# aynik/carta1

Measured on AMD Instinct MI355X. Metric: atrac1_stereo_frames_per_s_encode, higher is better.
Workload: dtype f32+f64

## Files before the change

### carta1_amd/csrc/c1_k_allocate.hip

```cpp
#include "c1_device.h"

namespace {

constexpr int kHeapSlotsPerLane = 52 + 1;
constexpr uint32_t kLow = 0x1FFFFFu;
constexpr uint32_t kSentinel = 52u;
constexpr int kCandBytes = kCandidateBytes;
constexpr double kAlive = -1.0;

__device__ __forceinline__ uint32_t heap_entry(uint32_t rank, int size, int s, int wl, int b) {
  return (rank << 21) | ((uint32_t)size << 16) | ((uint32_t)s << 10) | ((uint32_t)wl << 6) | (uint32_t)b;
}

__device__ __forceinline__ void heap_sift_down(uint32_t *hp, int sentinel, int i, uint32_t v, uint32_t el,
                                               uint32_t er, bool active) {
  const uint32_t vmax = v | kLow;
  for (;;) {
    const uint32_t m = max(el | kLow, vmax);
    const bool take_r = er > m;
    const bool take_l = !take_r && el > vmax;
    const bool moved = active && (take_r || take_l);
    if (active) hp[i * 64] = moved ? (take_r ? er : el) : v;
    active = moved;
    if (__builtin_amdgcn_ballot_w64(active) == 0) break;
    i = moved ? 2 * i + 1 + (take_r ? 1 : 0) : i;
    const int l = 2 * i + 1;
    const uint32_t *src = hp + min(l, sentinel - 1) * 64;
    el = l < sentinel ? src[0] : 0u;
    er = src[64];
  }
}

constexpr int kSpecsHost[52] = {8, 8, 8, 8, 4, 4, 4, 4, 8, 8, 8, 8, 6, 6, 6, 6, 6, 6, 6, 6, 6, 6, 6, 6, 7, 7, 7, 7, 9, 9, 9, 9, 10, 10, 10, 10,
                                12, 12, 12, 12, 12, 12, 12, 12, 20, 20, 20, 20, 20, 20, 20, 20};
constexpr int dist_class(int size) {
  for (int c = 0; c < 8; c++) if (kDistSizes[c] == size) return c;
  return -1;
}
constexpr bool sizes_come_in_fours() {
  for (int b = 0; b < 52; b++) if (kSpecsHost[b] != kSpecsHost[b & ~3]) return false;
  return true;
}
static_assert(sizes_come_in_fours(), "the four BFUs whose indices share a dword share a size");
static_assert(dist_class(4) == 0 && dist_class(20) == 7 && dist_class(kSpecsHost[24]) == 2, "every BFU size has its row of the distortion tables");

__device__ __forceinline__ void reopen(uint32_t (&sf)[13]) {
#pragma unroll
  for (int i = 0; i < 13; i++) asm volatile("" : "+v"(sf[i]));
}

template <bool AFFINE>
__device__ __forceinline__ void heap_phase(uint32_t *hp, int n, const uint32_t (&sf)[13], const C1DevEncOpts *O, bool live) {
  const __attribute__((address_space(4))) uint16_t *rank_t = (const __attribute__((address_space(4))) uint16_t *)O->rank;
  const uint32_t mul0 = ((uint32_t)O->rank_a << 11) | 1u, add0 = (uint32_t)(O->rank_c + O->rank_off) << 11;
  const uint32_t step0 = O->rank_step0, step = O->rank_step;
  int remaining = 212 * 8 - 40 - 10 * n;
  int hs = 0;
#pragma unroll
  for (int b0 = 0; b0 < 52; b0 += 13) if (own_block()) {
#pragma unroll
  for (int b = b0; b < b0 + 13; b++) {
    if (b < n) {
      const int s = (sf[b >> 2] >> ((b & 3) * 8)) & 63;
      const uint32_t fixed = ((uint32_t)kSpecsHost[b] << 16) | (uint32_t)b;
      if constexpr (AFFINE) hp[hs * 64] = ((__umul24(mul0, (uint32_t)s) + add0) << 10) | fixed;
      else hp[hs * 64] = ((uint32_t)rank_t[s * 16] << 21) | ((uint32_t)s << 10) | fixed;
      hs += (s != 0 && live) ? 1 : 0;
    }
  }
  }
  for (int k = hs; k < kHeapSlotsPerLane; k++) hp[k * 64] = kSentinel;
  for (int i = (hs >> 1) - 1; i >= 0; i--) {
    const int l = 2 * i + 1;
    heap_sift_down(hp, 52, i, hp[i * 64], hp[l * 64], hp[(l + 1) * 64], true);
  }
  uint32_t r0 = hp[0], r1 = hp[64], r2 = hp[128];
  bool run = remaining >= 4 && hs > 0;
  while (__builtin_amdgcn_ballot_w64(run) != 0) {
    const uint32_t top = r0;
    const bool wl0 = (top & (15u << 6)) == 0;
    const int size = (top >> 16) & 31;
    const int cost = size << (wl0 ? 1 : 0);
    const bool fits = cost <= remaining;
    uint32_t v, upd;
    bool last_wl;
    if constexpr (AFFINE) {
      v = top + (wl0 ? step0 : step);
      upd = (fits ? v : top) & kLow;
      last_wl = (v & (15u << 6)) == (15u << 6);
    } else {
      const int wl = (top >> 6) & 15, s = (top >> 10) & 63;
      const int nxt = wl + (fits ? 1 : 0);
      upd = (top & ~((0x3FFu << 21) | (15u << 6))) | ((uint32_t)nxt << 6);
      v = upd | ((uint32_t)rank_t[s * 16 + (nxt & 15)] << 21);
      last_wl = nxt >= 15;
    }
    const bool leaves = run && (!fits || last_wl);
    if (__builtin_amdgcn_ballot_w64(leaves) != 0) {
      const int li = hs - 1;
      const uint32_t deep = hp[(li > 3 ? li : 3) * 64];
      const uint32_t last = li == 0 ? r0 : (li == 1 ? r1 : (li == 2 ? r2 : deep));
      if (leaves) {
        v = last;
        hs = li;
        if (li > 2) hp[li * 64] = upd;
        r0 = li == 0 ? upd : r0; r1 = li == 1 ? upd : r1; r2 = li == 2 ? upd : r2;
      }
    }
    if (run) remaining -= fits ? cost : 0;
    const bool sift = run && hs > 0;
    const uint32_t vmax = v | kLow;
    const bool tr0 = r2 > max(r1 | kLow, vmax);
    const bool tl0 = !tr0 && r1 > vmax;
    const bool mv0 = sift && (tr0 || tl0);
    if (sift) r0 = mv0 ? (tr0 ? r2 : r1) : v;
    {
      const int i1 = tr0 ? 2 : 1;
      const uint32_t *src = hp + (2 * i1 + 1) * 64;
      const uint32_t el = src[0], er = src[64];
      const uint32_t g0 = src[(2 * i1 + 2) * 64], g1 = src[(2 * i1 + 3) * 64], g2 = src[(2 * i1 + 4) * 64], g3 = src[(2 * i1 + 5) * 64];
      const bool tr1 = er > max(el | kLow, vmax);
      const bool tl1 = !tr1 && el > vmax;
      const bool mv1 = mv0 && (tr1 || tl1);
      const uint32_t val = mv1 ? (tr1 ? er : el) : v;
      if (mv0) { if (tr0) r2 = val; else r1 = val; }
      {
        const int i2 = 2 * i1 + 1 + (tr1 ? 1 : 0);
        const uint32_t c0 = tr1 ? g2 : g0, c1 = tr1 ? g3 : g1;
        const bool tr2 = c1 > max(c0 | kLow, vmax);
        const bool tl2 = !tr2 && c0 > vmax;
        const bool mv2 = mv1 && (tr2 || tl2);
        if (mv1) hp[i2 * 64] = mv2 ? (tr2 ? c1 : c0) : v;
        if (__builtin_amdgcn_ballot_w64(mv2) != 0) {
          const int i3 = 2 * i2 + 1 + (tr2 ? 1 : 0);
          const uint32_t *s3 = hp + (2 * i3 + 1) * 64;
          const uint32_t d0 = s3[0], d1 = s3[64];
          const bool far = i3 >= 12;
          const uint32_t *s4 = hp + min(4 * i3 + 3, 49) * 64;
          const uint32_t h0 = s4[0], h1 = s4[64], h2 = s4[128], h3 = s4[192];
          const bool tr3 = d1 > max(d0 | kLow, vmax);
          const bool tl3 = !tr3 && d0 > vmax;
          const bool mv3 = mv2 && (tr3 || tl3);
          if (mv2) hp[i3 * 64] = mv3 ? (tr3 ? d1 : d0) : v;
          const int i4 = 2 * i3 + 1 + (tr3 ? 1 : 0);
          const bool upper = tr3 || far;
          const uint32_t e0 = upper ? h2 : h0, e1 = upper ? h3 : h1;
          const bool tr4 = e1 > max(e0 | kLow, vmax);
          const bool tl4 = !tr4 && e0 > vmax;
          const bool mv4 = mv3 && i4 < 26 && (tr4 || tl4);
          if (mv3) hp[i4 * 64] = mv4 ? (tr4 ? e1 : e0) : v;
          if (mv4) hp[(2 * i4 + 1 + (tr4 ? 1 : 0)) * 64] = v;
        }
      }
    }
    run = run && remaining >= 4 && hs > 0;
  }
  hp[0] = r0; hp[64] = r1; hp[128] = r2;
}

template <bool BOUND>
__device__ __forceinline__ void totals_tabled(int n, const uint32_t (&sf)[13], const C1DevEncOpts *O, uint64_t res0, uint64_t res1,
                                              uint64_t res2, uint64_t res3, double &total, double (&lbs)[7]) {
  typedef double d2 __attribute__((ext_vector_type(2)));
  const __attribute__((address_space(4))) d2 *dist = (const __attribute__((address_space(4))) d2 *)O->dist;
  total = 0.0;
#pragma unroll
  for (int c = 0; c < 7; c++) lbs[c] = 0.0;
#pragma unroll
  for (int b0 = 0; b0 < 52; b0 += 13) if (own_block()) {
#pragma unroll
  for (int b = b0; b < b0 + 13; b++) {
    const int s = (sf[b >> 2] >> ((b & 3) * 8)) & 63;
    const uint64_t word = b < 16 ? res0 : (b < 32 ? res1 : (b < 48 ? res2 : res3));
    const int wl = (int)((word >> ((b & 15) * 4)) & 15);
    const d2 zc = dist[dist_class(kSpecsHost[b]) * 64 + s];
    const double coded = __hiloint2double(__double2hiint(zc.y) - ((wl + 1) << 20), __double2loint(zc.y));
    total += (b >= n || wl == 0) ? zc.x : coded;
    if constexpr (BOUND) {
      if (b >= 20) lbs[0] += zc.x;
      if (b >= 28) lbs[1] += zc.x;
      if (b >= 32) lbs[2] += zc.x;
      if (b >= 36) lbs[3] += zc.x;
      if (b >= 40) lbs[4] += zc.x;
      if (b >= 44) lbs[5] += zc.x;
      if (b >= 48) lbs[6] += zc.x;
    }
  }
  }
}

template <bool BOUND>
__device__ __forceinline__ void totals_direct(int n, const uint32_t (&sf)[13], const C1DevEncOpts *O, uint64_t res0, uint64_t res1,
                                              uint64_t res2, uint64_t res3, double &total, double (&lbs)[7]) {
  const __attribute__((address_space(4))) double *biased = (const __attribute__((address_space(4))) double *)O->biased;
  total = 0.0;
#pragma unroll
  for (int c = 0; c < 7; c++) lbs[c] = 0.0;
#pragma unroll
  for (int b0 = 0; b0 < 52; b0 += 13) if (own_block()) {
#pragma unroll
  for (int b = b0; b < b0 + 13; b++) {
    const int s = (sf[b >> 2] >> ((b & 3) * 8)) & 63;
    const uint64_t word = b < 16 ? res0 : (b < 32 ? res1 : (b < 48 ? res2 : res3));
    const int wl = (int)((word >> ((b & 15) * 4)) & 15);
    const int size = kSpecsHost[b];
    const double bs = biased[s];
    const double z = s != 0 ? (double)f32(bs * 2.0 * (double)size) : 0.0;
    const double ip2 = __hiloint2double((1023 - wl_bits(wl)) << 20, 0);
    const double coded = s != 0 ? bs * ip2 * (double)size : 0.0;
    total += (b >= n || wl == 0) ? z : coded;
    if constexpr (BOUND) {
      if (b >= 20) lbs[0] += z;
      if (b >= 28) lbs[1] += z;
      if (b >= 32) lbs[2] += z;
      if (b >= 36) lbs[3] += z;
      if (b >= 40) lbs[4] += z;
      if (b >= 44) lbs[5] += z;
      if (b >= 48) lbs[6] += z;
    }
  }
  }
}

template <bool BOUND>
__device__ __forceinline__ void run_candidate(uint32_t *hp, int n, uint32_t (&sf)[13], const C1DevEncOpts *O,
                                              bool live, uint64_t &res0, uint64_t &res1, uint64_t &res2,
                                              uint64_t &res3, double &total, double (&lbs)[7]) {
  if (O->rank_affine != 0) heap_phase<true>(hp, n, sf, O, live);
  else heap_phase<false>(hp, n, sf, O, live);
  {
    uint8_t *hb = reinterpret_cast<uint8_t *>(hp);
#pragma unroll
    for (int k = 0; k < 52; k++) hb[k * 256 + 3] = 0;
#pragma unroll
    for (int k0 = 0; k0 < 52; k0 += 8) {
      uint32_t e[8];
#pragma unroll
      for (int j = 0; j < 8; j++) if (k0 + j < 52) e[j] = hp[(k0 + j) * 64];
#pragma unroll
      for (int j = 0; j < 8; j++) if (k0 + j < 52) hb[(e[j] & 63u) * 256 + 3] = (uint8_t)((e[j] >> 6) & 15u);
    }
    uint32_t d[8];
#pragma unroll
    for (int i = 0; i < 8; i++) {
      d[i] = 0;
#pragma unroll
      for (int j = 0; j < 8; j++) if (8 * i + j < 52) d[i] |= (hp[(8 * i + j) * 64] >> 24) << (4 * j);
    }
    res0 = (uint64_t)d[0] | ((uint64_t)d[1] << 32); res1 = (uint64_t)d[2] | ((uint64_t)d[3] << 32);
    res2 = (uint64_t)d[4] | ((uint64_t)d[5] << 32); res3 = (uint64_t)d[6] | ((uint64_t)d[7] << 32);
  }
  reopen(sf);
  if (O->dist_tables != 0) totals_tabled<BOUND>(n, sf, O, res0, res1, res2, res3, total, lbs);
  else totals_direct<BOUND>(n, sf, O, res0, res1, res2, res3, total, lbs);
}

__device__ __forceinline__ void load_sfi(const uint8_t *side, int64_t unit, uint32_t (&sf)[13]) {
  const uint4 *src = reinterpret_cast<const uint4 *>(side + unit * kSideBytes);
  const uint4 a = src[0], b = src[1], c = src[2];
  const uint32_t d = reinterpret_cast<const uint32_t *>(src)[12];
  sf[0] = a.x; sf[1] = a.y; sf[2] = a.z; sf[3] = a.w; sf[4] = b.x; sf[5] = b.y; sf[6] = b.z; sf[7] = b.w;
  sf[8] = c.x; sf[9] = c.y; sf[10] = c.z; sf[11] = c.w; sf[12] = d;
}

__device__ __forceinline__ void store_candidate(uint8_t *cand, int64_t unit, int c, double total, uint64_t r0,
                                                uint64_t r1, uint64_t r2, uint64_t r3) {
  uint8_t *base = cand + unit * kCandBytes;
  reinterpret_cast<double *>(base)[c] = total;
  uint64_t *dst = reinterpret_cast<uint64_t *>(base + 64 + c * 32);
  dst[0] = r0; dst[1] = r1; dst[2] = r2; dst[3] = r3;
}

__device__ __forceinline__ bool getenv_no_tonal(const C1DevEncOpts *O) { return O->alloc_no_tonal != 0; }

__global__ __launch_bounds__(C1_WAVE, 3) void k_alloc_first(C1EncodeLaunch L) {
  __shared__ uint32_t heap[kHeapSlotsPerLane * 64];
  const C1DevEncOpts *O = L.opts;
  const __attribute__((address_space(4))) double *biased = (const __attribute__((address_space(4))) double *)O->biased;
  const int lane = threadIdx.x;
  const bool listed = L.unit_list != nullptr;
  const int64_t units_total = listed ? (int64_t)*L.unit_count : L.frames * L.channels;
  for (int64_t pos0 = (int64_t)blockIdx.x * 64; pos0 < units_total; pos0 += (int64_t)gridDim.x * 64) {
  const int64_t pos = pos0 + lane;
  const bool live = pos < units_total;
  const int64_t unit = listed ? (int64_t)L.unit_list[live ? pos : 0] : pos;
  uint32_t sf[13];
  load_sfi(L.side, live ? unit : 0, sf);
  bool tonal = false;
  {
    uint32_t n_int = 0, s_int = 0;
#pragma unroll
    for (int g = 0; g < 13; g++) {
      const uint32_t x = sf[g] & 0x3F3F3F3Fu;
      const uint32_t nz = ((x + 0x3F3F3F3Fu) >> 6) & 0x01010101u;
      n_int = __umul24(__builtin_amdgcn_sad_u8(nz, 0u, 0u), (uint32_t)kSpecsHost[4 * g]) + n_int;
      s_int = __umul24(__builtin_amdgcn_sad_u8(x, 0u, 0u), (uint32_t)kSpecsHost[4 * g]) + s_int;
    }
    const float n_coef = (float)n_int, s_la = (float)s_int;
    const float la_sum = __builtin_fmaf(O->la_slope, s_la, O->la_off * n_coef);
    const float t_est = 1.442695f * n_coef * __builtin_amdgcn_exp2f((la_sum - 1136.0f) / n_coef);
    float t6f = 0.0f;
#pragma unroll
    for (int b = 48; b < 52; b++) {
      const int s = (sf[b >> 2] >> ((b & 3) * 8)) & 63;
      const float bs = (float)biased[s];
      t6f += s != 0 ? bs * (2.0f * (float)kSpecsHost[b]) : 0.0f;
    }
    const bool mine = n_coef > 0.0f && t6f < 0.35f * t_est && !getenv_no_tonal(O);
    tonal = 2 * __popcll(__builtin_amdgcn_ballot_w64(live && mine)) > __popcll(__builtin_amdgcn_ballot_w64(live));
  }
  uint64_t r0, r1, r2, r3;
  double total;
  double lbs[7];
  reopen(sf);
  run_candidate<true>(heap + lane, 52, sf, O, live && !tonal, r0, r1, r2, r3, total, lbs);
  uint32_t survivors = 0;
  {
    const double t0 = lbs[0], t1 = lbs[1], t2 = lbs[2], t3 = lbs[3], t4 = lbs[4], t5 = lbs[5], t6 = lbs[6];
    const bool finite = total < __builtin_huge_val();
    survivors = (!(finite && t0 > total) ? 1u : 0u) | (!(finite && t1 > total) ? 2u : 0u) |
                (!(finite && t2 > total) ? 4u : 0u) | (!(finite && t3 > total) ? 8u : 0u) |
                (!(finite && t4 > total) ? 16u : 0u) | (!(finite && t5 > total) ? 32u : 0u) |
                (!(finite && t6 > total) ? 64u : 0u);
  }
  if (tonal) survivors = 0xffu;
  const bool finite52 = total < __builtin_huge_val();
  if (live && survivors == 0) {
    uint64_t *dst = reinterpret_cast<uint64_t *>(L.alloc + unit * kAllocBytes);
    if (finite52) { dst[0] = r0; dst[1] = r1; dst[2] = r2; dst[3] = r3 | (7ull << 60); }
    else { dst[0] = 0; dst[1] = 0; dst[2] = 0; dst[3] = 1ull << 59; }
  } else if (live) {
    uint8_t *base = L.cand + unit * kCandBytes;
    double *tot = reinterpret_cast<double *>(base);
#pragma unroll
    for (int c = 0; c < 7; c++) tot[c] = ((survivors >> c) & 1u) ? kAlive : __builtin_huge_val();
    if (tonal) tot[7] = kAlive;
    else store_candidate(L.cand, unit, 7, finite52 ? total : __builtin_huge_val(), r0, r1, r2, r3);
  }
  const uint64_t sel_mask = __builtin_amdgcn_ballot_w64(live && survivors != 0);
  uint32_t sel_base = 0;
  if (lane == 0 && sel_mask != 0) sel_base = atomicAdd(L.work_count + 1, (uint32_t)__popcll(sel_mask));
  sel_base = (uint32_t)__builtin_amdgcn_readfirstlane((int)sel_base);
  if (live && survivors != 0) L.sel_list[sel_base + (uint32_t)__popcll(sel_mask & ((1ull << lane) - 1ull))] = (uint32_t)unit;
  }
}

typedef _Float16 h2 __attribute__((ext_vector_type(2)));
__global__ __launch_bounds__(256) void k_alloc_bound(C1EncodeLaunch L) {
  __shared__ double biased_s[64];
  const C1DevEncOpts *O = L.opts;
  if (threadIdx.x < 64) biased_s[threadIdx.x] = threadIdx.x == 0 ? 0.0 : ((const __attribute__((address_space(4))) double *)O->biased)[threadIdx.x];
  __syncthreads();
  const float la_slope = O->la_slope, la_off = O->la_off;
  const int lane = threadIdx.x & 63;
  const uint32_t count = L.work_count[1];
  for (uint32_t pos0 = blockIdx.x * 256u; pos0 < count; pos0 += gridDim.x * 256u) {
    const uint32_t pos = pos0 + threadIdx.x;
    const bool live = pos < count;
    const int64_t unit = live ? (int64_t)L.sel_list[pos] : (int64_t)L.sel_list[0];
    uint32_t sf[13];
    load_sfi(L.side, unit, sf);
    uint8_t *base = L.cand + unit * kCandBytes;
    double *tot = reinterpret_cast<double *>(base);
    double *lb = reinterpret_cast<double *>(base + kCandLbOffset);
    const double t52 = tot[7];
    const double best = t52 == kAlive ? __builtin_huge_val() : t52;
    int smin = 64, smax = 0;
#pragma unroll
    for (int b = 0; b < 52; b++) {
      const int s = (sf[b >> 2] >> ((b & 3) * 8)) & 63;
      if (s != 0) { smin = s < smin ? s : smin; smax = s > smax ? s : smax; }
    }
    h2 sp[26];
#pragma unroll
    for (int k = 0; k < 26; k++) {
      const int s0 = (sf[(2 * k) >> 2] >> (((2 * k) & 3) * 8)) & 63, s1 = (sf[(2 * k + 1) >> 2] >> (((2 * k + 1) & 3) * 8)) & 63;
      sp[k] = h2{s0 != 0 ? (_Float16)s0 : (_Float16)-1000.0f, s1 != 0 ? (_Float16)s1 : (_Float16)-1000.0f};
    }
    const h2 slope2 = h2{(_Float16)la_slope, (_Float16)la_slope};
    float x_prev = 0.0f;
    bool have_prev = false;
    int c_star = -1;
    double lb_star = __builtin_huge_val();
    for (int c = 0; c < 8; c++) {
      const bool mine = live && tot[c] == kAlive;
      if (__builtin_amdgcn_ballot_w64(mine) == 0) continue;
      const int n = bfu_amount(c);
      const int B = 212 * 8 - 40 - 10 * n;
      float lo = have_prev ? x_prev - 0.05f : __builtin_fmaf(la_slope, (float)smin, la_off) - 17.0f;
      float hi = have_prev ? x_prev + 3.15f : __builtin_fmaf(la_slope, (float)smax, la_off);
      const int iters = __builtin_amdgcn_ballot_w64(mine && !have_prev) != 0 ? 8 : 5;
      for (int it = 0; it < iters; it++) {
        const float x = 0.5f * (lo + hi);
        const _Float16 by = (_Float16)(la_off - x - 0.5f);
        const h2 base2 = h2{by, by};
        float used = 0.0f;
#pragma unroll
        for (int k = 0; k < 26; k++) {
          if (2 * k < n) {
            const h2 y = __builtin_elementwise_fma(sp[k], slope2, base2);
            const h2 bits = __builtin_elementwise_min(__builtin_elementwise_max(y, h2{(_Float16)2.0f, (_Float16)2.0f}), h2{(_Float16)16.0f, (_Float16)16.0f});
            const h2 ramp = __builtin_elementwise_fma(y, h2{(_Float16)64.0f, (_Float16)64.0f}, h2{(_Float16)20.0f, (_Float16)20.0f});
            const h2 on = __builtin_elementwise_min(__builtin_elementwise_max(ramp, h2{(_Float16)0.0f, (_Float16)0.0f}), h2{(_Float16)1.0f, (_Float16)1.0f});
            used = __builtin_amdgcn_fdot2(bits * on, h2{(_Float16)(float)kSpecsHost[2 * k], (_Float16)(float)kSpecsHost[2 * k + 1]}, used, false);
          }
        }
        if (used > (float)B) lo = x; else hi = x;
      }
      const float x = hi;
      const double lambda = (double)__builtin_amdgcn_exp2f(x);
      const double inv_lambda = 1.0 / lambda;
      double P = 0.0;
#pragma unroll
      for (int b = 0; b < 52; b++) {
        const int s = (sf[b >> 2] >> ((b & 3) * 8)) & 63;
        const double a = biased_s[s], size = (double)kSpecs[b];
        const double z = (double)f32(a * 2.0 * size);
        double g = z;
        if (b < n) {
          const double q = a * inv_lambda;
          int e = ((__double2hiint(q) >> 20) & 0x7ff) - 1023;
          e = e < 2 ? 2 : (e > 16 ? 16 : e);
          const double ip2 = __hiloint2double((1023 - e) << 20, 0);
          const double h = a * ip2 * size + lambda * size * (double)e;
          g = h < z ? h : z;
        }
        P += g;
      }
      const double M = lambda * (double)B;
      const double bound = (P - M) - 5.684341886080802e-14 * (P + M);
      if (mine) {
        if (bound > best) tot[c] = __builtin_huge_val();
        else {
          lb[c] = bound;
          if (bound < lb_star || c_star < 0) { lb_star = bound; c_star = c; }
        }
        x_prev = x; have_prev = true;
      }
    }
    const bool has = live && c_star >= 0;
    const uint64_t m = __builtin_amdgcn_ballot_w64(has);
    uint32_t at = 0;
    if (lane == 0 && m != 0) at = atomicAdd(L.work_count, (uint32_t)__popcll(m));
    at = (uint32_t)__builtin_amdgcn_readfirstlane((int)at);
    if (has) L.work_list[at + (uint32_t)__popcll(m & ((1ull << lane) - 1ull))] = ((uint32_t)unit << 3) | (uint32_t)c_star;
  }
}

template <bool FIRST_ROUND>
__global__ __launch_bounds__(C1_WAVE, 3) void k_alloc_rest(C1EncodeLaunch L, const uint32_t *__restrict__ list, const uint32_t *__restrict__ list_count,
                                                           uint32_t *__restrict__ list2) {
  __shared__ uint32_t heap[kHeapSlotsPerLane * 64];
  const C1DevEncOpts *O = L.opts;
  const int lane = threadIdx.x;
  const uint32_t count = *list_count;
  for (uint32_t base = blockIdx.x * 64u; base < count; base += gridDim.x * 64u) {
    const uint32_t idx = base + lane;
    const bool live = idx < count;
    const uint32_t item = live ? list[idx] : 0u;
    const int64_t unit = item >> 3;
    const int c = item & 7;
    uint32_t sf[13];
    load_sfi(L.side, unit, sf);
    uint64_t r0, r1, r2, r3;
    double total;
    double unused[7];
    run_candidate<false>(heap + lane, bfu_amount(c), sf, O, live, r0, r1, r2, r3, total, unused);
    total = total < __builtin_huge_val() ? total : __builtin_huge_val();
    if (live) store_candidate(L.cand, unit, c, total, r0, r1, r2, r3);
    if constexpr (FIRST_ROUND) {
      uint8_t *cbase = L.cand + unit * kCandBytes;
      double *tot = reinterpret_cast<double *>(cbase);
      const double *lb = reinterpret_cast<const double *>(cbase + kCandLbOffset);
      uint32_t keep = 0;
      if (live) {
        const double t52 = tot[7];
        const double best = (c == 7 || t52 == kAlive || total < t52) ? total : t52;
#pragma unroll
        for (int k = 0; k < 8; k++) {
          if (k != c && tot[k] == kAlive) {
            if (lb[k] > best) tot[k] = __builtin_huge_val();
            else keep |= 1u << k;
          }
        }
      }
      const int mine = __popc(keep);
      const int scan = wave_inclusive_scan(mine);
      const int wave_total = __builtin_amdgcn_readlane(scan, 63);
      uint32_t at = 0;
      if (lane == 0 && wave_total > 0) at = atomicAdd(L.work_count + 2, (uint32_t)wave_total);
      at = (uint32_t)__builtin_amdgcn_readfirstlane((int)at) + (uint32_t)(scan - mine);
      for (int k = 0; k < 8; k++)
        if ((keep >> k) & 1u) list2[at++] = ((uint32_t)unit << 3) | (uint32_t)k;
    }
  }
}

__global__ __launch_bounds__(256) void k_alloc_select(C1EncodeLaunch L) {
  const int64_t count = (int64_t)L.work_count[1];
  for (int64_t pos = (int64_t)blockIdx.x * 256 + threadIdx.x; pos < count; pos += (int64_t)gridDim.x * 256) {
  const int64_t unit = (int64_t)L.sel_list[pos];
  const uint8_t *base = L.cand + unit * kCandBytes;
  const double *tot = reinterpret_cast<const double *>(base);
  double best = __builtin_huge_val();
  int best_c = 8;
#pragma unroll
  for (int c = 0; c < 8; c++) {
    const double t = tot[c];
    if (t < best) { best = t; best_c = c; }
  }
  uint64_t *dst = reinterpret_cast<uint64_t *>(L.alloc + unit * kAllocBytes);
  if (best_c < 8) {
    const uint64_t *src = reinterpret_cast<const uint64_t *>(base + 64 + best_c * 32);
    dst[0] = src[0]; dst[1] = src[1]; dst[2] = src[2];
    dst[3] = src[3] | ((uint64_t)best_c << 60);
  } else {
    dst[0] = 0; dst[1] = 0; dst[2] = 0;
    dst[3] = 1ull << 59;
  }
  }
}

__global__ __launch_bounds__(256) void k_alloc_tap_init(C1EncodeLaunch L, int64_t units) {
  const int64_t unit = (int64_t)blockIdx.x * 256 + threadIdx.x;
  if (unit == 0) { L.work_count[0] = 0; L.work_count[1] = (uint32_t)units; L.work_count[2] = (uint32_t)(units * 8); }
  if (unit >= units) return;
  double *tot = reinterpret_cast<double *>(L.cand + unit * kCandBytes);
  for (int c = 0; c < 7; c++) tot[c] = kAlive;
  tot[7] = __builtin_huge_val();
  L.sel_list[unit] = (uint32_t)unit;
  for (int c = 0; c < 8; c++) L.work_list[units + unit * 8 + c] = ((uint32_t)unit << 3) | (uint32_t)c;
}
__global__ __launch_bounds__(256) void k_alloc_tap_gather(C1EncodeLaunch L, int64_t units, double *out) {
  const int64_t unit = (int64_t)blockIdx.x * 256 + threadIdx.x;
  if (unit >= units) return;
  const double *tot = reinterpret_cast<const double *>(L.cand + unit * kCandBytes);
  const double *lb = reinterpret_cast<const double *>(L.cand + unit * kCandBytes + kCandLbOffset);
  for (int c = 0; c < 8; c++) { out[unit * 16 + c] = tot[c]; out[unit * 16 + 8 + c] = c < 7 ? lb[c] : 0.0; }
  const uint32_t a7 = reinterpret_cast<const uint32_t *>(L.alloc + unit * kAllocBytes)[7];
  out[unit * 16 + 15] = ((a7 >> 27) & 1u) ? -1.0 : (double)((a7 >> 28) & 7u);
}

}

void c1k_launch_alloc_tap(const C1EncodeLaunch &L, double *out, hipStream_t stream) {
  const int64_t units = L.frames * L.channels;
  c1k_launch_allocate(L, stream);
  const dim3 grid((unsigned)((units + 255) / 256)), block(256);
  hipLaunchKernelGGL(k_alloc_tap_init, grid, block, 0, stream, L, units);
  hipLaunchKernelGGL(k_alloc_bound, dim3((unsigned)std::min<int64_t>((units + 255) / 256, 2048)), block, 0, stream, L);
  hipLaunchKernelGGL((k_alloc_rest<false>), dim3((unsigned)std::min<int64_t>((units * 8 + 63) / 64, 256 * 10)), dim3(C1_WAVE), 0, stream, L,
                     (const uint32_t *)(L.work_list + units), (const uint32_t *)(L.work_count + 2), (uint32_t *)nullptr);
  hipLaunchKernelGGL(k_alloc_tap_gather, grid, block, 0, stream, L, units, out);
}

namespace {
}

void c1k_launch_allocate(const C1EncodeLaunch &L, hipStream_t stream) {
  const int64_t units = L.frames * L.channels;
  const bool listed = L.unit_list != nullptr;
  (void)hipMemsetAsync(L.work_count, 0, 3 * sizeof(uint32_t), stream);
  const int64_t first_blocks = listed ? std::min<int64_t>((units + 63) / 64, 256 * 12) : (units + 63) / 64;
  hipLaunchKernelGGL(k_alloc_first, dim3((unsigned)first_blocks), dim3(C1_WAVE), 0, stream, L);
  const int64_t unit_blocks = std::min<int64_t>((units + 255) / 256, 2048);
  uint32_t *list2 = L.work_list + units;
  hipLaunchKernelGGL(k_alloc_bound, dim3((unsigned)unit_blocks), dim3(256), 0, stream, L);
  const int64_t rest1_blocks = std::min<int64_t>((units + 63) / 64, 256 * 10);
  hipLaunchKernelGGL((k_alloc_rest<true>), dim3((unsigned)rest1_blocks), dim3(C1_WAVE), 0, stream, L, (const uint32_t *)L.work_list, (const uint32_t *)L.work_count, list2);
  const int64_t rest2_blocks = std::min<int64_t>((units * 6 + 63) / 64, 256 * 10);
  hipLaunchKernelGGL((k_alloc_rest<false>), dim3((unsigned)rest2_blocks), dim3(C1_WAVE), 0, stream, L, (const uint32_t *)list2, (const uint32_t *)(L.work_count + 2), (uint32_t *)nullptr);
  const int64_t select_blocks = std::min<int64_t>((units + 255) / 256, 1024);
  hipLaunchKernelGGL(k_alloc_select, dim3((unsigned)select_blocks), dim3(256), 0, stream, L);
}
```

Measured before the change: 196.9 million.

## Keep heap top three entries in registers and shrink per-lane LDS heap

The bit-allocation heap now stores only entries from index 3 onward in LDS; the root and its two children stay in registers for the whole heap build and pop loop. This cuts the LDS footprint per single-wave workgroup from 53 rows to 50, aiming to fit more workgroups per CU. The sift-down path is restructured to defer writing the moving value until its final hole is known, which removes repeated stores. The word-length extraction is also changed to pack nibbles into spare heap bytes. The price is more complex index arithmetic and some added branching during heapify.

```diff
diff --git a/carta1_amd/csrc/c1_k_allocate.hip b/carta1_amd/csrc/c1_k_allocate.hip
--- a/carta1_amd/csrc/c1_k_allocate.hip
+++ b/carta1_amd/csrc/c1_k_allocate.hip
@@ -2,7 +2,9 @@
 
 namespace {
 
-constexpr int kHeapSlotsPerLane = 52 + 1;
+constexpr int kHeapRows = 52 - 3 + 1;
+constexpr int kHeapLdsBytes = kHeapRows * 64 * 4;
+static_assert((kHeapLdsBytes + 1279) / 1280 * 12 <= 128, "heaps: 12 single-wave workgroups per CU = at most 10 LDS blocks of 1 280 bytes each");
 constexpr uint32_t kLow = 0x1FFFFFu;
 constexpr uint32_t kSentinel = 52u;
 constexpr int kCandBytes = kCandidateBytes;
@@ -12,23 +14,36 @@
   return (rank << 21) | ((uint32_t)size << 16) | ((uint32_t)s << 10) | ((uint32_t)wl << 6) | (uint32_t)b;
 }
 
-__device__ __forceinline__ void heap_sift_down(uint32_t *hp, int sentinel, int i, uint32_t v, uint32_t el,
-                                               uint32_t er, bool active) {
+__device__ __forceinline__ void heap_sift_down(uint32_t *hp, int i, uint32_t v, uint32_t el, uint32_t er, bool active) {
   const uint32_t vmax = v | kLow;
   for (;;) {
     const uint32_t m = max(el | kLow, vmax);
     const bool take_r = er > m;
     const bool take_l = !take_r && el > vmax;
     const bool moved = active && (take_r || take_l);
-    if (active) hp[i * 64] = moved ? (take_r ? er : el) : v;
+    if (active) hp[(i - 3) * 64] = moved ? (take_r ? er : el) : v;
     active = moved;
     if (__builtin_amdgcn_ballot_w64(active) == 0) break;
     i = moved ? 2 * i + 1 + (take_r ? 1 : 0) : i;
     const int l = 2 * i + 1;
-    const uint32_t *src = hp + min(l, sentinel - 1) * 64;
-    el = l < sentinel ? src[0] : 0u;
+    const uint32_t *src = hp + (min(l, 51) - 3) * 64;
+    el = l < 52 ? src[0] : 0u;
     er = src[64];
   }
+}
+
+__device__ __forceinline__ uint32_t heap_sift_below_root(uint32_t *hp, int k, uint32_t v, bool active) {
+  const uint32_t *src = hp + (2 * k - 2) * 64;
+  const uint32_t el = src[0], er = src[64];
+  const uint32_t vmax = v | kLow;
+  const bool take_r = er > max(el | kLow, vmax);
+  const bool take_l = !take_r && el > vmax;
+  const bool moved = active && (take_r || take_l);
+  if (__builtin_amdgcn_ballot_w64(moved) != 0) {
+    const int i = 2 * k + 1 + (take_r ? 1 : 0);
+    heap_sift_down(hp, i, v, hp[(2 * i + 1 - 3) * 64], hp[(2 * i + 2 - 3) * 64], moved);
+  }
+  return moved ? (take_r ? er : el) : v;
 }
 
 constexpr int kSpecsHost[52] = {8, 8, 8, 8, 4, 4, 4, 4, 8, 8, 8, 8, 6, 6, 6, 6, 6, 6, 6, 6, 6, 6, 6, 6, 7, 7, 7, 7, 9, 9, 9, 9, 10, 10, 10, 10,
@@ -50,33 +65,65 @@
 }
 
 template <bool AFFINE>
-__device__ __forceinline__ void heap_phase(uint32_t *hp, int n, const uint32_t (&sf)[13], const C1DevEncOpts *O, bool live) {
+__device__ __forceinline__ void heap_phase(uint32_t *hp, int n, const uint32_t (&sf)[13], const C1DevEncOpts *O, bool live,
+                                           uint32_t &r0, uint32_t &r1, uint32_t &r2) {
   const __attribute__((address_space(4))) uint16_t *rank_t = (const __attribute__((address_space(4))) uint16_t *)O->rank;
   const uint32_t mul0 = ((uint32_t)O->rank_a << 11) | 1u, add0 = (uint32_t)(O->rank_c + O->rank_off) << 11;
   const uint32_t step0 = O->rank_step0, step = O->rank_step;
   int remaining = 212 * 8 - 40 - 10 * n;
-  int hs = 0;
+  uint32_t cur = 47;
 #pragma unroll
   for (int b0 = 0; b0 < 52; b0 += 13) if (own_block()) {
 #pragma unroll
-  for (int b = b0; b < b0 + 13; b++) {
+  for (int b = b0; b < b0 + 13 && b < 50; b++) {
     if (b < n) {
       const int s = (sf[b >> 2] >> ((b & 3) * 8)) & 63;
       const uint32_t fixed = ((uint32_t)kSpecsHost[b] << 16) | (uint32_t)b;
-      if constexpr (AFFINE) hp[hs * 64] = ((__umul24(mul0, (uint32_t)s) + add0) << 10) | fixed;
-      else hp[hs * 64] = ((uint32_t)rank_t[s * 16] << 21) | ((uint32_t)s << 10) | fixed;
+      uint32_t *at = hp + min(cur, cur - (uint32_t)kHeapRows) * 64;
+      if constexpr (AFFINE) *at = ((__umul24(mul0, (uint32_t)s) + add0) << 10) | fixed;
+      else *at = ((uint32_t)rank_t[s * 16] << 21) | ((uint32_t)s << 10) | fixed;
+      cur += (s != 0 && live) ? 1 : 0;
+    }
+  }
+  }
+  int hs = (int)cur - 47;
+  r0 = hp[47 * 64]; r1 = hp[48 * 64]; r2 = hp[49 * 64];
+#pragma unroll
+  for (int b = 50; b < 52; b++) {
+    if (b < n) {
+      const int s = (sf[b >> 2] >> ((b & 3) * 8)) & 63;
+      const uint32_t fixed = ((uint32_t)kSpecsHost[b] << 16) | (uint32_t)b;
+      uint32_t e;
+      if constexpr (AFFINE) e = ((__umul24(mul0, (uint32_t)s) + add0) << 10) | fixed;
+      else e = ((uint32_t)rank_t[s * 16] << 21) | ((uint32_t)s << 10) | fixed;
+      r0 = hs == 0 ? e : r0; r1 = hs == 1 ? e : r1; r2 = hs == 2 ? e : r2;
+      if (hs >= 3) hp[(hs - 3) * 64] = e;
       hs += (s != 0 && live) ? 1 : 0;
     }
   }
-  }
-  for (int k = hs; k < kHeapSlotsPerLane; k++) hp[k * 64] = kSentinel;
-  for (int i = (hs >> 1) - 1; i >= 0; i--) {
+  r0 = hs > 0 ? r0 : kSentinel; r1 = hs > 1 ? r1 : kSentinel; r2 = hs > 2 ? r2 : kSentinel;
+  for (int k = max(hs, 3) - 3; k < kHeapRows; k++) hp[k * 64] = kSentinel;
+  const int half = hs >> 1;
+  for (int i = half - 1; i >= 3; i--) {
     const int l = 2 * i + 1;
-    heap_sift_down(hp, 52, i, hp[i * 64], hp[l * 64], hp[(l + 1) * 64], true);
-  }
-  uint32_t r0 = hp[0], r1 = hp[64], r2 = hp[128];
-  bool run = remaining >= 4 && hs > 0;
-  while (__builtin_amdgcn_ballot_w64(run) != 0) {
+    heap_sift_down(hp, i, hp[(i - 3) * 64], hp[(l - 3) * 64], hp[(l - 2) * 64], true);
+  }
+  if (__builtin_amdgcn_ballot_w64(half >= 2) != 0) {
+    r2 = heap_sift_below_root(hp, 2, r2, half >= 3);
+    r1 = heap_sift_below_root(hp, 1, r1, half >= 2);
+  }
+  if (__builtin_amdgcn_ballot_w64(half >= 1) != 0) {
+    const uint32_t v = r0, vmax = v | kLow;
+    const bool take_r = r2 > max(r1 | kLow, vmax);
+    const bool take_l = !take_r && r1 > vmax;
+    const bool moved = half >= 1 && (take_r || take_l);
+    r0 = moved ? (take_r ? r2 : r1) : v;
+    const uint32_t below = heap_sift_below_root(hp, take_r ? 2 : 1, v, moved);
+    r1 = (moved && !take_r) ? below : r1; r2 = (moved && take_r) ? below : r2;
+  }
+  remaining = hs > 0 ? remaining : 0;
+  while (__builtin_amdgcn_ballot_w64(remaining >= 4) != 0) {
+    const bool run = remaining >= 4;
     const uint32_t top = r0;
     const bool wl0 = (top & (15u << 6)) == 0;
     const int size = (top >> 16) & 31;
@@ -95,67 +142,66 @@
       v = upd | ((uint32_t)rank_t[s * 16 + (nxt & 15)] << 21);
       last_wl = nxt >= 15;
     }
+    remaining -= fits ? cost : 0;
     const bool leaves = run && (!fits || last_wl);
-    if (__builtin_amdgcn_ballot_w64(leaves) != 0) {
+    if (__builtin_expect(__builtin_amdgcn_ballot_w64(leaves) != 0, 0)) {
       const int li = hs - 1;
-      const uint32_t deep = hp[(li > 3 ? li : 3) * 64];
-      const uint32_t last = li == 0 ? r0 : (li == 1 ? r1 : (li == 2 ? r2 : deep));
+      const uint32_t deep = hp[(max(li, 3) - 3) * 64];
       if (leaves) {
-        v = last;
+        v = li == 0 ? upd : (li == 1 ? r1 : (li == 2 ? r2 : deep));
         hs = li;
-        if (li > 2) hp[li * 64] = upd;
-        r0 = li == 0 ? upd : r0; r1 = li == 1 ? upd : r1; r2 = li == 2 ? upd : r2;
+        if (li > 2) hp[(li - 3) * 64] = upd;
+        r1 = li == 1 ? upd : r1; r2 = li == 2 ? upd : r2;
+        remaining = li == 0 ? 0 : remaining;
       }
     }
-    if (run) remaining -= fits ? cost : 0;
-    const bool sift = run && hs > 0;
     const uint32_t vmax = v | kLow;
-    const bool tr0 = r2 > max(r1 | kLow, vmax);
-    const bool tl0 = !tr0 && r1 > vmax;
-    const bool mv0 = sift && (tr0 || tl0);
-    if (sift) r0 = mv0 ? (tr0 ? r2 : r1) : v;
-    {
-      const int i1 = tr0 ? 2 : 1;
-      const uint32_t *src = hp + (2 * i1 + 1) * 64;
-      const uint32_t el = src[0], er = src[64];
-      const uint32_t g0 = src[(2 * i1 + 2) * 64], g1 = src[(2 * i1 + 3) * 64], g2 = src[(2 * i1 + 4) * 64], g3 = src[(2 * i1 + 5) * 64];
-      const bool tr1 = er > max(el | kLow, vmax);
-      const bool tl1 = !tr1 && el > vmax;
-      const bool mv1 = mv0 && (tr1 || tl1);
-      const uint32_t val = mv1 ? (tr1 ? er : el) : v;
-      if (mv0) { if (tr0) r2 = val; else r1 = val; }
-      {
-        const int i2 = 2 * i1 + 1 + (tr1 ? 1 : 0);
-        const uint32_t c0 = tr1 ? g2 : g0, c1 = tr1 ? g3 : g1;
-        const bool tr2 = c1 > max(c0 | kLow, vmax);
-        const bool tl2 = !tr2 && c0 > vmax;
-        const bool mv2 = mv1 && (tr2 || tl2);
-        if (mv1) hp[i2 * 64] = mv2 ? (tr2 ? c1 : c0) : v;
-        if (__builtin_amdgcn_ballot_w64(mv2) != 0) {
-          const int i3 = 2 * i2 + 1 + (tr2 ? 1 : 0);
-          const uint32_t *s3 = hp + (2 * i3 + 1) * 64;
-          const uint32_t d0 = s3[0], d1 = s3[64];
-          const bool far = i3 >= 12;
-          const uint32_t *s4 = hp + min(4 * i3 + 3, 49) * 64;
-          const uint32_t h0 = s4[0], h1 = s4[64], h2 = s4[128], h3 = s4[192];
-          const bool tr3 = d1 > max(d0 | kLow, vmax);
-          const bool tl3 = !tr3 && d0 > vmax;
-          const bool mv3 = mv2 && (tr3 || tl3);
-          if (mv2) hp[i3 * 64] = mv3 ? (tr3 ? d1 : d0) : v;
-          const int i4 = 2 * i3 + 1 + (tr3 ? 1 : 0);
-          const bool upper = tr3 || far;
-          const uint32_t e0 = upper ? h2 : h0, e1 = upper ? h3 : h1;
-          const bool tr4 = e1 > max(e0 | kLow, vmax);
-          const bool tl4 = !tr4 && e0 > vmax;
-          const bool mv4 = mv3 && i4 < 26 && (tr4 || tl4);
-          if (mv3) hp[i4 * 64] = mv4 ? (tr4 ? e1 : e0) : v;
-          if (mv4) hp[(2 * i4 + 1 + (tr4 ? 1 : 0)) * 64] = v;
-        }
-      }
-    }
-    run = run && remaining >= 4 && hs > 0;
-  }
-  hp[0] = r0; hp[64] = r1; hp[128] = r2;
+    const bool t0 = r2 > (r1 | kLow);
+    const uint32_t w0 = t0 ? r2 : r1;
+    const bool mv0 = run && w0 > vmax;
+    if (run) r0 = mv0 ? w0 : v;
+    const uint32_t *s1 = hp + (t0 ? 2 : 0) * 64;
+    const uint32_t el = s1[0], er = s1[64];
+    const uint32_t *s2 = hp + (t0 ? 8 : 4) * 64;
+    const uint32_t g0 = s2[0], g1 = s2[64], g2 = s2[128], g3 = s2[192];
+    const bool t1 = er > (el | kLow);
+    const uint32_t w1 = t1 ? er : el;
+    const bool mv1 = mv0 && w1 > vmax;
+    const uint32_t val = mv1 ? w1 : v;
+    r1 = (mv0 && !t0) ? val : r1; r2 = (mv0 && t0) ? val : r2;
+    const uint32_t cl = t1 ? g2 : g0, cr = t1 ? g3 : g1;
+    const bool t2 = cr > (cl | kLow);
+    const uint32_t w2 = t2 ? cr : cl;
+    const bool mv2 = mv1 && w2 > vmax;
+    const int q2 = (t0 ? 2 : 0) + (t1 ? 1 : 0);
+    uint32_t *hole = hp + q2 * 64;
+    if (mv2) *hole = w2;
+    if (__builtin_amdgcn_ballot_w64(mv2) != 0) {
+      const int q3 = 2 * q2 + 4 + (t2 ? 1 : 0);
+      const uint32_t *s3 = hp + (2 * q3 + 4) * 64;
+      const uint32_t d0 = s3[0], d1 = s3[64];
+      const bool far = q3 >= 9;
+      const uint32_t *s4 = hp + min(4 * q3 + 12, kHeapRows - 4) * 64;
+      const uint32_t h0 = s4[0], h1 = s4[64], h2 = s4[128], h3 = s4[192];
+      const bool t3 = d1 > (d0 | kLow);
+      const uint32_t w3 = t3 ? d1 : d0;
+      const bool mv3 = mv2 && w3 > vmax;
+      uint32_t *p3 = hp + q3 * 64;
+      hole = mv2 ? p3 : hole;
+      if (mv3) *p3 = w3;
+      const int q4 = 2 * q3 + 4 + (t3 ? 1 : 0);
+      const bool upper = t3 || far;
+      const uint32_t e0 = upper ? h2 : h0, e1 = upper ? h3 : h1;
+      const bool t4 = e1 > (e0 | kLow);
+      const uint32_t w4 = t4 ? e1 : e0;
+      const bool mv4 = mv3 && q4 < 23 && w4 > vmax;
+      uint32_t *p4 = hp + q4 * 64;
+      hole = mv3 ? p4 : hole;
+      if (mv4) *p4 = w4;
+      hole = mv4 ? hp + (2 * q4 + 4 + (t4 ? 1 : 0)) * 64 : hole;
+    }
+    if (mv1) *hole = v;
+  }
 }
 
 template <bool BOUND>
@@ -226,26 +272,30 @@
 __device__ __forceinline__ void run_candidate(uint32_t *hp, int n, uint32_t (&sf)[13], const C1DevEncOpts *O,
                                               bool live, uint64_t &res0, uint64_t &res1, uint64_t &res2,
                                               uint64_t &res3, double &total, double (&lbs)[7]) {
-  if (O->rank_affine != 0) heap_phase<true>(hp, n, sf, O, live);
-  else heap_phase<false>(hp, n, sf, O, live);
+  uint32_t top[3];
+  if (O->rank_affine != 0) heap_phase<true>(hp, n, sf, O, live, top[0], top[1], top[2]);
+  else heap_phase<false>(hp, n, sf, O, live, top[0], top[1], top[2]);
   {
     uint8_t *hb = reinterpret_cast<uint8_t *>(hp);
-#pragma unroll
-    for (int k = 0; k < 52; k++) hb[k * 256 + 3] = 0;
-#pragma unroll
-    for (int k0 = 0; k0 < 52; k0 += 8) {
+    auto put = [hb](uint32_t e) { hb[((e & 62u) << 7) + (e & 1u) + 2] = (uint8_t)((e >> 6) & 15u); };
+#pragma unroll
+    for (int k = 0; k < 26; k++) *reinterpret_cast<uint16_t *>(hb + k * 256 + 2) = 0;
+#pragma unroll
+    for (int j = 0; j < 3; j++) put(top[j]);
+#pragma unroll
+    for (int k0 = 0; k0 < kHeapRows - 1; k0 += 8) {
       uint32_t e[8];
 #pragma unroll
-      for (int j = 0; j < 8; j++) if (k0 + j < 52) e[j] = hp[(k0 + j) * 64];
-#pragma unroll
-      for (int j = 0; j < 8; j++) if (k0 + j < 52) hb[(e[j] & 63u) * 256 + 3] = (uint8_t)((e[j] >> 6) & 15u);
+      for (int j = 0; j < 8; j++) if (k0 + j < kHeapRows - 1) e[j] = hp[(k0 + j) * 64];
+#pragma unroll
+      for (int j = 0; j < 8; j++) if (k0 + j < kHeapRows - 1) put(e[j]);
     }
     uint32_t d[8];
 #pragma unroll
     for (int i = 0; i < 8; i++) {
       d[i] = 0;
 #pragma unroll
-      for (int j = 0; j < 8; j++) if (8 * i + j < 52) d[i] |= (hp[(8 * i + j) * 64] >> 24) << (4 * j);
+      for (int j = 0; j < 8; j++) if (8 * i + j < 52) d[i] |= (uint32_t)hb[((8 * i + j) >> 1) * 256 + 2 + (j & 1)] << (4 * j);
     }
     res0 = (uint64_t)d[0] | ((uint64_t)d[1] << 32); res1 = (uint64_t)d[2] | ((uint64_t)d[3] << 32);
     res2 = (uint64_t)d[4] | ((uint64_t)d[5] << 32); res3 = (uint64_t)d[6] | ((uint64_t)d[7] << 32);
@@ -274,7 +324,7 @@
 __device__ __forceinline__ bool getenv_no_tonal(const C1DevEncOpts *O) { return O->alloc_no_tonal != 0; }
 
 __global__ __launch_bounds__(C1_WAVE, 3) void k_alloc_first(C1EncodeLaunch L) {
-  __shared__ uint32_t heap[kHeapSlotsPerLane * 64];
+  __shared__ uint32_t heap[kHeapRows * 64];
   const C1DevEncOpts *O = L.opts;
   const __attribute__((address_space(4))) double *biased = (const __attribute__((address_space(4))) double *)O->biased;
   const int lane = threadIdx.x;
@@ -450,7 +500,7 @@
 template <bool FIRST_ROUND>
 __global__ __launch_bounds__(C1_WAVE, 3) void k_alloc_rest(C1EncodeLaunch L, const uint32_t *__restrict__ list, const uint32_t *__restrict__ list_count,
                                                            uint32_t *__restrict__ list2) {
-  __shared__ uint32_t heap[kHeapSlotsPerLane * 64];
+  __shared__ uint32_t heap[kHeapRows * 64];
   const C1DevEncOpts *O = L.opts;
   const int lane = threadIdx.x;
   const uint32_t count = *list_count;
```

New measurement: 202.0 million (median of 6 runs). +2.6%, better.
